# GrokImageCompression/Grok

Measured on AMD Instinct MI355X. Metric: encode Mpixels/s (whole node), 8K RGB HTJ2K lossless, higher is better.
Workload: dtype int16x2 packed (exact: range-proven on the host, int32 fallback); 1 GPU; 8192x8192x3 8-bit RGB, 1 tile, RCT+5/3 lossless HTJ2K, 5 levels, 64x64 blocks (BASELINE metric shape); tiles_per_gpu=1, code_blocks_per_gpu=49152, packed_dwt_levels=4, generator=G2 (SURVEY.md §8d), parallelism=1 GPU, consecutive encodes pipelined (grk_amd_set_pipelining), prewarm_steps=40, input_frames_in_rotation=3

## Files before the change

grok_amd/csrc/context.h:

```cpp
#pragma once
#include "../../include/grok_amd.h"
#include "geometry.h"
#include "kernels.h"
#include "pixel_layout.h"
#include <hip/hip_runtime.h>
#include <cstdio>
#include <cstdlib>
#include <cstring>
#include <string>
#include <vector>
#include <algorithm>
#include <cmath>
#include <atomic>
#include <thread>

using namespace grk_amd;

#pragma GCC visibility push(hidden)
struct DevBuf {
    void* p = nullptr;
    size_t cap = 0;
    hipError_t ensure(size_t n)
    {
        if (n <= cap) return hipSuccess;
// ... 61 lines not shown
    grk_amd_tile_params gp{};
    bool have_geom = false;
    TileGeom geom;
    std::vector<HtBlockDesc> h_desc, h_desc_dec;
    std::vector<uint16_t> dec_qcd;
    std::vector<float> dec_steps;
    std::vector<uint32_t> dec_seg_first;
    std::vector<grk_amd_segment> dec_segs;
    grk_amd_pixel_layout enc_layout{};
    grk_amd_pixel_layout dec_layout{};
    bool dec_upsample = false;
    uint32_t dec_reduce = 0;
    std::vector<uint32_t> red_seg_first;
    std::vector<grk_amd_segment> red_segs;
    DevBuf dec_seg_dev;
    std::vector<HtClassPlan> ht_classes;
    int seq_index = -1;
    int seq_flavour = 0;
    hipStream_t side2 = nullptr; hipEvent_t ev_side2 = nullptr;
    hipStream_t side = nullptr;
    hipEvent_t ev_level0 = nullptr, ev_side = nullptr;
    bool overlap = false;
    static constexpr int kMaxAltSets = 7;
    struct AltSet { DevBuf p1, arena, lengths, offsets, flag, ovf, llA, llB; hipEvent_t ev_side = nullptr, ev_side2 = nullptr; } alts[kMaxAltSets];
    int alt_head = 0;
    int pipe_depth = 2;
    DevBuf ovf;
    bool lds_cap = true;
    bool pipelining = false;
    hipEvent_t ev_main = nullptr;
    bool side_pending = false;
    bool dec_planes16 = true;
    int dwt_pk = 1;
    bool k3_alternate = true;
    uint32_t num_cus = 0;
    uint32_t k3_parity = 0;
    int dwt_xcd = 1;
    bool fuse_egress = true;
    bool planes16 = true;
    DevBuf ht_sel;
    DevBuf energy;
    struct T2State {
        bool valid = false; grk_amd_tile_params p{}; uint32_t order = 0;
        T2Plan plan; uint32_t max_blocks = 0;
        DevBuf packets, pob;
    } t2;
    DevBuf t2_u, t2_h, t2_rel, t2_pkhdr, t2_pkbody, t2_pkdst, t2_lit, t2_litlen, t2_index;
    struct T2Out { DevBuf out, tile_dst, part_len, total; };
    T2Out t2_outs[kMaxAltSets + 1];
    int t2_cur = 0;
    uint64_t t2_out_used = 0;
    std::vector<uint64_t> h_off;
    std::vector<uint32_t> h_len;
    uint32_t last_ntiles = 0;
    uint64_t last_nblocks = 0;
    bool last_h16 = false;
    const uint8_t* last_drops = nullptr;
    DevBuf drops_keep;
    DevBuf rate_L, rate_E, rate_W, rate_drop, rate_res, rate_map, rate_bdrop;
    struct RateState { bool valid = false; RatePlan plan{}; uint64_t nblocks = 0; uint32_t ntiles = 0; std::vector<uint64_t> unit_rows;
                       uint64_t budget = 0;  } rate;
    HostStage stage;
    void* d2h_pin = nullptr; size_t d2h_cap = 0; std::vector<hipEvent_t> d2h_ev;
    hipEvent_t ev_dec_front = nullptr, ev_dec_top = nullptr;
    bool dec_top_pending = false;
    int frame_streams = 1; int fs_parity = 0;
// ... 121 lines not shown
```

grok_amd/csrc/context.hip:

```cpp
#include "context.h"

namespace {
bool create_alt_events(grk_amd_ctx* c)
{
    for (auto& as : c->alts)
        if (hipEventCreateWithFlags(&as.ev_side, hipEventDisableTiming) != hipSuccess ||
            hipEventCreateWithFlags(&as.ev_side2, hipEventDisableTiming) != hipSuccess) return false;
    return true;
}

#ifndef GRK_AMD_OVERLAP_DEFAULT
#define GRK_AMD_OVERLAP_DEFAULT 1
#endif

void drain_timers(grk_amd_ctx* c)
{
    for (auto& t : c->timers) {
        for (auto& pr : t.ev) {
            float ms = 0;
            if (hipEventSynchronize(pr.second) == hipSuccess && hipEventElapsedTime(&ms, pr.first, pr.second) == hipSuccess) {
                t.total_ms += ms; t.launches++;
            }
            (void)hipEventDestroy(pr.first); (void)hipEventDestroy(pr.second);
        }
// ... 175 lines not shown
    c->have_geom = true;
    return GRK_AMD_OK;
}

int stage_enter(grk_amd_ctx* c, const grk_amd_tile_params* p, bool args_ok, bool join, const char* refuse)
{
    if (c && join) { const int jr = join_side(c); if (jr) return jr; }
    if (!c || !p || !args_ok) return GRK_AMD_ERR_INVALID;
    if (refuse) return fail(c, GRK_AMD_ERR_INVALID, refuse);
    HIP_TRY(c, hipSetDevice(c->device), "set device");
    return ensure_geom(c, p);
}

int create_context(int device_id, int verbose, bool decode_only, grk_amd_ctx** out)
{
    if (!out) return GRK_AMD_ERR_INVALID;
    *out = nullptr;
    int n = 0;
    if (hipGetDeviceCount(&n) != hipSuccess || n <= 0) return GRK_AMD_ERR_NO_DEVICE;
    if (device_id < 0 || device_id >= n) return GRK_AMD_ERR_INVALID;
    if (hipSetDevice(device_id) != hipSuccess) return GRK_AMD_ERR_NO_DEVICE;
    auto* c = new grk_amd_ctx();
    c->device = device_id; c->verbose = verbose;
    { int cus = 0; if (hipDeviceGetAttribute(&cus, hipDeviceAttributeMultiprocessorCount, device_id) == hipSuccess && cus > 0) c->num_cus = (uint32_t)cus; }
    if (hipStreamCreateWithFlags(&c->stream, hipStreamNonBlocking) != hipSuccess) { delete c; return GRK_AMD_ERR_NO_DEVICE; }
    c->own_stream = true;
    {
        int least = 0, greatest = 0;
        (void)hipDeviceGetStreamPriorityRange(&least, &greatest);
        if (const char* e16 = getenv("GRK_AMD_PLANES16")) c->planes16 = atoi(e16) != 0;
        if (const char* ef = getenv("GRK_AMD_FUSE_EGRESS")) c->fuse_egress = atoi(ef) != 0;
        if (const char* ex = getenv("GRK_AMD_DWT_XCD")) c->dwt_xcd = atoi(ex) != 0;
        if (const char* ex = getenv("GRK_AMD_DWT_PK")) c->dwt_pk = atoi(ex) != 0;
        if (const char* ek = getenv("GRK_AMD_K3_ALT")) c->k3_alternate = atoi(ek) != 0;
        if (const char* ed = getenv("GRK_AMD_DEC_PLANES16")) c->dec_planes16 = atoi(ed) != 0;
        if (const char* el = getenv("GRK_AMD_LDS_CAP")) c->lds_cap = atoi(el) != 0;
        if (const char* ef2 = getenv("GRK_AMD_FRAME_STREAMS")) c->frame_streams = atoi(ef2);
        if (const char* et = getenv("GRK_AMD_T1_LANES")) c->t1_lanes = atoi(et);
        if (const char* ey = getenv("GRK_AMD_T1_SYNC")) c->t1_pass_sync = atoi(ey) != 0;
        if (const char* ep = getenv("GRK_AMD_STREAM_PROBE")) c->stream_probe = atoi(ep);
        c->side_priority = least;
        const char* e = getenv("GRK_AMD_OVERLAP");
        c->overlap = e ? atoi(e) != 0 : GRK_AMD_OVERLAP_DEFAULT;
        if (hipStreamCreateWithPriority(&c->side, hipStreamNonBlocking, least) != hipSuccess ||
            (!decode_only && hipStreamCreateWithPriority(&c->side2, hipStreamNonBlocking, least) != hipSuccess) ||
            hipEventCreateWithFlags(&c->ev_side2, hipEventDisableTiming) != hipSuccess ||
            !create_alt_events(c) ||
            hipEventCreateWithFlags(&c->ev_level0, hipEventDisableTiming) != hipSuccess ||
            hipEventCreateWithFlags(&c->ev_side, hipEventDisableTiming) != hipSuccess) {
            c->side = nullptr; c->overlap = false;
        }
    }
    *out = c;
    return GRK_AMD_OK;
}

extern "C" {
const char* grk_amd_version(void) { return "grok_amd 0.1 (gfx950)"; }

int grk_amd_create(int device_id, int verbose, grk_amd_ctx** out) { return create_context(device_id, verbose, false, out); }

void grk_amd_destroy(grk_amd_ctx* c)
{
    if (!c) return;
    for (grk_amd_ctx* k : c->dec_kids) grk_amd_destroy(k);
    c->dec_kids.clear();
// ... 180 lines not shown
```

grok_amd/csrc/dwt_instances.h:

```cpp
#pragma once
#include <cstdint>

namespace grk_amd {

struct LevelPart { uint32_t comp0, zdiv, nc; };
inline bool     level_has_triple(bool mct, uint32_t ncomp) { return mct && ncomp >= 3; }
inline uint32_t level_part_count(bool mct, uint32_t ncomp) { return level_has_triple(mct, ncomp) ? ncomp - 2 : 1; }
inline LevelPart level_part(bool mct, uint32_t ncomp, uint32_t i)
{
    if (!level_has_triple(mct, ncomp)) return LevelPart{0, ncomp, 1};
    return i == 0 ? LevelPart{0, 1, 3} : LevelPart{i + 2, 1, 1};
}
inline uint32_t level_part_zslots(bool mct, uint32_t ncomp) { return level_has_triple(mct, ncomp) ? 1u : ncomp; }

inline uint32_t row_segment_pairs(uint64_t strips, uint32_t row_pairs, uint32_t zslots, uint32_t min_wgs)
{
    uint32_t seg = 64;
    while (seg > 8 && strips * ((row_pairs + seg - 1) / seg) * zslots < min_wgs) seg >>= 1;
    return seg;
}

struct DwtKey {
    bool f97; uint8_t nc, px; bool h16, gen, str;
    constexpr uint32_t code() const { return (uint32_t)f97 | nc << 1 | px << 4 | (uint32_t)h16 << 6 | (uint32_t)gen << 7 | (uint32_t)str << 8; }
};
struct DwtPkKey {
    uint8_t nc, px; uint16_t nt; uint8_t ch;
    constexpr uint32_t code() const { return nc | px << 3 | ch << 5 | (uint32_t)nt << 8; }
};
struct IdwtKey {
    bool f97; uint8_t nc, pxo; bool h16, str;
    constexpr uint32_t code() const { return (uint32_t)f97 | nc << 1 | pxo << 4 | (uint32_t)h16 << 6 | (uint32_t)str << 7; }
};
struct IdwtPkKey {
    uint8_t nc, pxo, ch;
    constexpr uint32_t code() const { return nc | pxo << 3 | ch << 5; }
};
struct EgressKey {
    uint8_t bytes, nc; bool str;
    constexpr uint32_t code() const { return bytes | nc << 3 | (uint32_t)str << 6; }
};
struct DwtInstance  { bool packed; DwtKey k; DwtPkKey pk; };
struct IdwtInstance { bool packed; IdwtKey k; IdwtPkKey pk; uint32_t grid_x; };

#define GRK_DWT_INSTANCES(X)                                                                      \
    X(true, 1, 0, false, true, false) X(false, 1, 0, true, true, false) X(false, 1, 0, false, true, false)                       \
    X(true, 3, 1, false, true, true) X(true, 3, 2, false, true, true) X(true, 1, 1, false, true, true) X(true, 1, 2, false, true, true) \
    X(false, 3, 1, true, true, true) X(false, 1, 1, true, true, true)                                                             \
    X(false, 3, 1, false, true, true) X(false, 3, 2, false, true, true) X(false, 1, 1, false, true, true) X(false, 1, 2, false, true, true) \
    X(true, 3, 1, false, false, false) X(true, 3, 1, false, true, false) X(true, 3, 2, false, false, false) X(true, 3, 2, false, true, false) \
    X(true, 1, 1, false, false, false) X(true, 1, 1, false, true, false) X(true, 1, 2, false, false, false) X(true, 1, 2, false, true, false) \
    X(false, 3, 1, true, true, false) X(false, 1, 1, true, true, false)                                                           \
    X(false, 3, 1, false, false, false) X(false, 3, 1, false, true, false) X(false, 3, 2, false, false, false) X(false, 3, 2, false, true, false) \
    X(false, 1, 1, false, false, false) X(false, 1, 1, false, true, false) X(false, 1, 2, false, false, false) X(false, 1, 2, false, true, false)
#define GRK_DWT_PK_INSTANCES(X)                                                                               \
    X(1, 0, 128, 0) X(1, 0, 256, 0)                                                                                               \
    X(1, 1, 128, 1) X(1, 1, 256, 1) X(3, 1, 128, 3) X(3, 1, 256, 3) X(1, 1, 128, 3) X(1, 1, 256, 3)                               \
    X(3, 1, 128, 4) X(3, 1, 256, 4) X(1, 1, 128, 4) X(1, 1, 256, 4)                                                               \
    X(3, 1, 128, 0) X(1, 1, 128, 0) X(3, 1, 256, 0) X(1, 1, 256, 0)
#define GRK_IDWT_INSTANCES(X)                                                                         \
    X(true, 1, 0, false, false) X(false, 1, 0, true, false) X(false, 1, 0, false, false)                                          \
    X(true, 3, 1, false, true) X(true, 3, 2, false, true) X(true, 1, 1, false, true) X(true, 1, 2, false, true)                   \
    X(true, 3, 1, false, false) X(true, 3, 2, false, false) X(true, 1, 1, false, false) X(true, 1, 2, false, false)               \
    X(false, 3, 1, true, true) X(false, 3, 2, true, true) X(false, 1, 1, true, true) X(false, 1, 2, true, true)                   \
    X(false, 3, 1, false, true) X(false, 3, 2, false, true) X(false, 1, 1, false, true) X(false, 1, 2, false, true)               \
    X(false, 3, 1, true, false) X(false, 3, 2, true, false) X(false, 1, 1, true, false) X(false, 1, 2, true, false)               \
    X(false, 3, 1, false, false) X(false, 3, 2, false, false) X(false, 1, 1, false, false) X(false, 1, 2, false, false)
#define GRK_IDWT_PK_INSTANCES(X)                                                                                 \
    X(1, 0, 0) X(1, 1, 1) X(3, 1, 3) X(3, 1, 4) X(3, 1, 0) X(1, 1, 0)
#define GRK_EGRESS_INSTANCES(X)                                                                               \
    X(1, 1, true) X(1, 2, true) X(1, 3, true) X(1, 4, true) X(2, 1, true) X(2, 2, true) X(2, 3, true) X(2, 4, true)               \
    X(1, 1, false) X(1, 2, false) X(1, 3, false) X(1, 4, false) X(2, 1, false) X(2, 2, false) X(2, 3, false) X(2, 4, false)       \
    X(4, 1, false) X(4, 2, false) X(4, 3, false) X(4, 4, false)

#define GRK_INSTANCE_ROW(...) {__VA_ARGS__},
inline constexpr DwtKey    kDwtInstances[]    = {GRK_DWT_INSTANCES(GRK_INSTANCE_ROW)};
inline constexpr DwtPkKey  kDwtPkInstances[]  = {GRK_DWT_PK_INSTANCES(GRK_INSTANCE_ROW)};
inline constexpr IdwtKey   kIdwtInstances[]   = {GRK_IDWT_INSTANCES(GRK_INSTANCE_ROW)};
inline constexpr IdwtPkKey kIdwtPkInstances[] = {GRK_IDWT_PK_INSTANCES(GRK_INSTANCE_ROW)};
inline constexpr EgressKey kEgressInstances[] = {GRK_EGRESS_INSTANCES(GRK_INSTANCE_ROW)};

}
```

grok_amd/csrc/encode.hip:

```cpp
#include "context.h"

namespace {
int encode_layout(grk_amd_ctx* c, uint32_t ntiles, PixelLayout& px)
{
    const char* why = "";
    if (!resolve_pixel_layout(c->geom.p, &c->enc_layout, 0, 0, ntiles, px, &why)) return fail(c, GRK_AMD_ERR_INVALID, why);
    return GRK_AMD_OK;
}

int run_ingest(grk_amd_ctx* c, uint32_t ntiles, const void* d_pixels, void* d_planes, const PixelLayout& px)
{
    const TileGeom& g = c->geom;
    const SampleRange r = sample_range(g.p);
    IngestArgs a{};
    set_px_in(a, px);
    a.pixels = d_pixels; a.planes = (int32_t*)d_planes;
    a.w = g.p.tile_w; a.h = g.p.tile_h; a.stride = g.stride; a.pitch = g.plane_elems;
    a.ncomp = g.p.num_comps; a.ntiles = ntiles;
    a.bytes_per_sample = r.bytes;
    a.dc = r.dc; a.sext = r.sext;
    a.mct = g.p.mct; a.irreversible = g.p.irreversible;
    ScopedTimer t(c, 0);
    HIP_TRY(c, launch_ingest(a, c->stream), "launch ingest");
    return GRK_AMD_OK;
// ... 49 lines not shown
int run_dwt(grk_amd_ctx* c, uint32_t nplanes, void* d_in, void* d_out, const void* d_pixels = nullptr, uint32_t ntiles = 0,
            const HtArgs* overlap_ht = nullptr, bool h16 = false, const PixelLayout* px = nullptr)
{
    const TileGeom& g = c->geom;
    const uint32_t L = g.p.num_levels;
    if (L == 0) {
        HIP_TRY(c, hipMemcpyAsync(d_out, d_in, (size_t)nplanes * g.plane_elems * 4, hipMemcpyDeviceToDevice, c->stream), "copy planes");
        return GRK_AMD_OK;
    }
    { const int rc = ensure_ll(c, nplanes); if (rc) return rc; }
    ScopedTimer t(c, 1);
    const SampleRange r = sample_range(g.p);
    for (uint32_t l = 0; l < L; ++l) {
        DwtLevelArgs a{};
        a.cw = level_geom(g, l).w; a.ch = level_geom(g, l).h;
        a.px = level_geom(g, l).x0 & 1u; a.py = level_geom(g, l).y0 & 1u;
        const LLPlane from = ll_plane(c, l, d_in, d_out), to = ll_plane(c, l + 1, d_in, d_out);
        a.in = (const int32_t*)from.p; a.in_stride = from.stride; a.in_pitch = from.pitch;
        a.mallat = (int32_t*)d_out; a.m_stride = g.stride; a.m_pitch = g.plane_elems;
        a.ll = (int32_t*)to.p; a.ll_stride = to.stride; a.ll_pitch = to.pitch;
        a.nplanes = nplanes;
        a.irreversible = g.p.irreversible;
        a.h16 = h16 ? 1 : 0;
        a.pk = h16 && c->dwt_pk && pk16_level_ok(g.p, l);
        a.xcd = c->dwt_xcd;
        if (l == 0 && d_pixels && px && px->lay) {
            set_px_in(a, *px); a.px_chan = px->channels;
        }
        const bool fused = l == 0 && d_pixels;
        const uint32_t zslots = fused ? ntiles * level_part_zslots(g.p.mct != 0, g.p.num_comps) : nplanes;
        const DwtLevelShape shape = plan_dwt_level(DwtLevelDesc{a.cw, a.ch, a.px, a.py, a.in_stride, a.m_stride, a.h16 != 0, a.pk != 0,
                                                                a.irreversible != 0, a.px_lay, a.px_chan, a.px_row, zslots, fused, r.bytes});
        a.seg_pairs = shape.seg_pairs;
        if (a.cw == 0 || a.ch == 0) {
        } else if (fused) {
            a.pixels = d_pixels; a.px_bytes = r.bytes;
            a.alloc_reset = c->pend_alloc; a.alloc_chunk_units = c->pend_alloc_units; c->pend_alloc = nullptr;
            a.dc = r.dc; a.sext = r.sext;
            HIP_TRY(c, launch_dwt_level0_fused(a, shape, ntiles, g.p.num_comps, g.p.mct, c->stream), "launch fused dwt level 0");
            if (c->want_px_event) HIP_TRY(c, hipEventRecord(c->ev_px, c->stream), "record the pixels' last read");
        } else {
            HIP_TRY(c, launch_dwt_level(a, shape, c->stream), "launch dwt level");
        }
        if (overlap_ht && (l == 0 || l + 1 == L)) {
            HIP_TRY(c, hipEventRecord(c->ev_level0, c->stream), "record level");
            const int rc = launch_ht_at(c, *overlap_ht, true, l == 0 ? HtPoint::AfterLevel0 : HtPoint::AfterLastLevel, L == 1);
            if (rc) return rc;
            if (l + 1 == L) {
                HIP_TRY(c, hipEventRecord(c->ev_side, c->side), "record side stream");
                HIP_TRY(c, hipEventRecord(c->ev_side2, c->side2), "record side stream 2");
            }
        }
    }
    return GRK_AMD_OK;
}

int run_ht(grk_amd_ctx* c, HtArgs a, bool overlapped = false, bool room = false)
{
    a.room = room ? 1 : 0;
    {
        ScopedTimer t(c, 2);
        if (!overlapped) HIP_TRY(c, launch_ht_alloc_init(a, c->stream), "reset arena allocator");
        const int rc = launch_ht_at(c, a, overlapped, HtPoint::RunHt, false);
        if (rc) return rc;
    }
    if (overlapped) {
        c->side_pending = true;
        if (!c->pipelining) { const int jr = join_side(c); if (jr) return jr; }
    }
    c->last_ntiles = a.ntiles;
    c->last_nblocks = (uint64_t)a.blocks_per_tile * a.ntiles;
    c->last_drops = nullptr;
    return GRK_AMD_OK;
}
}

int ht_encode_drops(grk_amd_ctx* c, uint32_t ntiles, const void* d_mallat, bool h16, const uint8_t* d_drops)
{
    HtArgs a;
    const int rc = make_ht_args(c, ntiles, d_mallat, h16, a); if (rc) return rc;
    const HtDropPlan dp = plan_ht_drop_instance(a.irreversible != 0, a.h16 != 0);
    if (!dp.ok) return fail(c, GRK_AMD_ERR_INVALID, "no encode keeps irreversible int16 planes");
    const uint64_t nblocks = (uint64_t)a.blocks_per_tile * a.ntiles;
    HIP_TRY(c, c->drops_keep.ensure(nblocks), "alloc drops copy");
    HIP_TRY(c, hipMemcpyAsync(c->drops_keep.p, d_drops, nblocks, hipMemcpyDeviceToDevice, c->stream), "keep the drops");
// ... 333 lines not shown
```

grok_amd/csrc/encode_constants.h:

```cpp
#pragma once
#include <cstddef>
#include <cstdint>

#if defined(__HIP_DEVICE_COMPILE__) || defined(__HIPCC__)
#define GRK_ENC_FN __host__ __device__ inline
#else
#define GRK_ENC_FN inline
#endif

namespace grk_amd {

constexpr uint32_t kHtMaxClasses = 24;
#ifndef GRK_HT_ALLOC_REGIONS
#define GRK_HT_ALLOC_REGIONS 64
#endif
constexpr uint32_t kHtAllocRegions = GRK_HT_ALLOC_REGIONS;
constexpr uint32_t kHtAllocChunk = 64u << 10;
constexpr uint32_t kHtAllocChunkSmall = 32u << 10;
constexpr size_t   kHtAllocBytes = 256u * (1u + kHtAllocRegions);
constexpr uint32_t kHtBlocksPerRegion = 64;
constexpr uint32_t kHtSmallJobBlocks = 16384;
constexpr size_t   kLdsPerCu = 160u << 10;
constexpr size_t   kMaxWavesPerCu = 32;
constexpr size_t   kLdsFor16Waves = 10240;

constexpr uint32_t kHtDropSkip = 0xFFu;
constexpr uint32_t kRateDefaultDrop = 6;
constexpr uint32_t kRateMaxDrop = 12;
constexpr uint32_t kRateMaxCand = kRateMaxDrop + 2;
constexpr uint32_t kRateAllocThreads = 1024;
constexpr uint32_t kRateBisectSteps = 40;
constexpr uint64_t kRateMaxBlocks = 0x7FFFFFFFull;
constexpr uint32_t kRateMaxRounds = 4;

constexpr uint64_t kFrameStreamSamples = 16ull << 20;

constexpr uint32_t kDwtStripCols = 448;
constexpr int      kPkLaneCols = 4;
constexpr uint32_t kPkNarrowCols = 2048;
GRK_ENC_FN uint32_t pk_strip_cols(uint32_t cw, uint32_t nt)
{
    const uint32_t most = ((nt - 2u) * kPkLaneCols) & ~63u;
    const uint32_t n = (cw + most - 1) / most;
    const uint32_t even = ((cw + n - 1) / n + 63u) & ~63u;
    return even < most ? even : most;
}
constexpr uint32_t kDwtMinWgsPacked = 2048;
constexpr uint32_t kDwtMinWgs = 4096;

}
```

grok_amd/csrc/encode_plan.cpp:

```cpp
#include "encode_plan.h"
#include <algorithm>

namespace grk_amd {

HtClasses plan_ht_classes(const TileGeom& g, uint32_t ncomp, bool lds_cap)
{
    HtClasses out;
    const uint32_t bpc = (uint32_t)g.blocks_comp0.size();
    auto add_class = [&](HtRole role, int top, int big) {
        HtClassPlan cl{0, 0, 0, 0, 0, (uint32_t)out.sel.size(), role};
        uint32_t hist[64] = {0};
        for (uint32_t i = 0; i < ncomp * bpc; ++i) {
            const grk_amd_block& b = g.blocks_comp0[i % bpc];
            if (top >= 0 && (int)(b.res == g.p.num_levels && g.p.num_levels >= 1) != top) continue;
            const uint32_t w = b.x1 - b.x0, h = b.y1 - b.y0;
            const uint32_t samples = w * h, quads = ((w + 1u) / 2u) * ((h + 1u) / 2u);
            if (big >= 0 && (int)(ht_lds_bytes(samples, quads, b.kmax) > kLdsFor16Waves) != big) continue;
            cl.count++;
            cl.max_kmax = std::max<uint32_t>(cl.max_kmax, b.kmax);
            cl.max_samples = std::max(cl.max_samples, samples);
            cl.max_quads = std::max(cl.max_quads, quads);
            hist[b.kmax & 63u] += samples;
            out.sel.push_back(i);
        }
// ... 154 lines not shown
    } else if (d.px_lay != 0) {
        in.packed = !d.irreversible && px == 1 && s.packed;
        const uint8_t ch = d.px_chan == 1 ? 1 : d.px_chan == 3 ? 3 : 4;
        in.pk = DwtPkKey{ch == 1 ? (uint8_t)1 : nc, 1, (uint16_t)s.lanes, ch};
        in.k = DwtKey{d.irreversible, nc, px, h16 && px == 1, true, true};
    } else {
        in.packed = !d.irreversible && px == 1 && s.packed;
        in.pk = DwtPkKey{nc, 1, (uint16_t)s.lanes, 0};
        if (h16 && px == 1) in.k = DwtKey{false, nc, 1, true, true, false};
        else                in.k = DwtKey{d.irreversible, nc, px, false, !s.all_fast, false};
    }
    return in;
}

DwtLevelShape plan_dwt_level(const DwtLevelDesc& d)
{
    DwtLevelShape s{};
    const bool near = (uint64_t)d.m_stride * d.ch < (1ull << 31) && (uint64_t)d.cw * d.ch < (1ull << 31) && (uint64_t)d.in_stride * d.ch < (1ull << 31);
    const bool lay = d.px_lay == 0 || (d.px_lay == 2 && (d.px_chan == 1 || d.px_chan == 3 || d.px_chan == 4) && d.px_row * d.ch < (1ull << 31));
    s.packed = d.h16 && d.pk && !d.irreversible && (d.px | d.py) == 0 && (d.cw & 3u) == 0 && d.cw >= 256u &&
               d.ch >= 16 && (d.ch & 1u) == 0 && near && lay;
    s.lanes = s.packed && d.cw <= kPkNarrowCols ? 128u : 256u;
    s.strip_cols = s.packed ? pk_strip_cols(d.cw, s.lanes) : kDwtStripCols;
    s.all_fast = (d.px | d.py) == 0 && (d.cw & 1u) == 0 && d.cw >= 4 && d.ch >= 16 && (d.ch & 1u) == 0;
    const uint32_t row_pairs = (d.ch + d.py + 1) >> 1;
    s.grid_x = (uint32_t)(((uint64_t)d.cw + d.px + s.strip_cols - 1) / s.strip_cols);
    s.seg_pairs = row_segment_pairs(s.grid_x, row_pairs, d.zslots, d.pk ? kDwtMinWgsPacked : kDwtMinWgs);
    s.grid_y = (row_pairs + s.seg_pairs - 1) / s.seg_pairs;
    s.inst[0] = dwt_instance(d, s, 1);
    if (d.fused) s.inst[1] = dwt_instance(d, s, 3);
    return s;
}

}
```

grok_amd/csrc/encode_plan.h:

```cpp
#pragma once
#include "dwt_instances.h"
#include "encode_constants.h"
#include "geometry.h"
#include <cstddef>
#include <cstdint>
#include <vector>

#pragma GCC visibility push(hidden)
namespace grk_amd {

enum class HtRole : uint8_t { Top, Rest, All, TopSmall, TopBig, RestSmall, RestBig };
struct HtClassPlan {
    uint32_t count;
    uint32_t max_kmax, max_samples, max_quads;
    uint32_t cap_kmax;
    uint32_t first;
    HtRole role;
};
struct HtClasses {
    std::vector<uint32_t> sel;
    std::vector<HtClassPlan> classes;
};
HtClasses plan_ht_classes(const TileGeom& g, uint32_t ncomp, bool lds_cap);

// ... 67 lines not shown
    bool overlap, pipelining; int frame_streams; bool planes16;
    bool have_side, have_side2;
    bool on_device;
    uint32_t px_align;
    uint64_t samples;
};
struct Route {
    bool fused;
    bool overlap;
    bool frame_stream;
    bool h16;
};
Route plan_route(const grk_amd_tile_params& p, const RouteIn& in);

struct DwtLevelDesc {
    uint32_t cw, ch, px, py;
    uint32_t in_stride, m_stride;
    bool h16, pk, irreversible;
    uint32_t px_lay, px_chan; uint64_t px_row;
    uint32_t zslots;
    bool fused; uint32_t px_bytes;
};
struct DwtLevelShape {
    bool packed;
    uint32_t lanes;
    uint32_t strip_cols;
    bool all_fast;
    uint32_t seg_pairs;
    uint32_t grid_x, grid_y;
    DwtInstance inst[2];
};
DwtLevelShape plan_dwt_level(const DwtLevelDesc& d);

}
#pragma GCC visibility pop
```

grok_amd/csrc/kernels.h:

```cpp
#pragma once
#include <cstdint>
#include <hip/hip_runtime.h>
#include "geometry.h"
#include "decode_constants.h"
#include "encode_constants.h"
#include "encode_plan.h"
#include "decode_plan.h"

namespace grk_amd {

struct IngestArgs {
    const void* pixels;
    int32_t*    planes;
    uint32_t w, h, stride;
    uint64_t pitch;
    uint32_t ncomp, ntiles;
    uint32_t bytes_per_sample;
    int32_t  dc;
    int32_t  sext;
    int      mct;
    int      irreversible;
    uint32_t px_lay, px_xstep;
    uint64_t px_row, px_kstep, px_tile;
};
hipError_t launch_ingest(const IngestArgs& a, hipStream_t s);

struct DwtLevelArgs {
    const int32_t* in;  uint32_t in_stride;  uint64_t in_pitch;
    int32_t* ll;        uint32_t ll_stride;  uint64_t ll_pitch;
    int32_t* mallat;    uint32_t m_stride;   uint64_t m_pitch;
    uint32_t cw, ch;
    uint32_t px, py;
    uint32_t nplanes;
    uint32_t seg_pairs;
    int      irreversible;
    const void* pixels;
    uint32_t px_bytes;
    int32_t  dc;
    int32_t  sext;
    uint32_t ncomp;
    uint32_t comp0, zdiv;
    unsigned long long* alloc_reset; uint32_t alloc_chunk_units;
    int      h16;
    int      xcd;
    int      pk;
    uint32_t px_lay, px_chan, px_xstep;
    uint64_t px_row, px_kstep, px_tile;
};
hipError_t launch_dwt_level(const DwtLevelArgs& a, const DwtLevelShape& sh, hipStream_t s);
hipError_t launch_dwt_level0_fused(const DwtLevelArgs& a0, const DwtLevelShape& sh, uint32_t ntiles, uint32_t ncomp, int mct, hipStream_t s);

struct HtBlockDesc {
    uint32_t px, py;
    uint16_t w, h;
    uint16_t comp;
    uint8_t  kmax;
    uint8_t  pad;
    float    inv_step;
};
struct HtClass {
    const uint32_t* sel;
    uint32_t count;
    uint32_t max_kmax, max_samples, max_quads;
    uint32_t ovf_base;
    uint32_t cap_kmax;
};
struct HtArgs {
    const int32_t* mallat; uint32_t stride; uint64_t pitch;
    int h16;
    int room;
    const HtBlockDesc* blocks; uint32_t blocks_per_tile; uint32_t ncomp; uint32_t ntiles;
    uint8_t*  arena; uint64_t arena_bytes;
    unsigned long long* alloc;
    uint32_t* lengths;
    unsigned long long* offsets;
    const uint32_t* sel; uint32_t sel_count;
    uint32_t* ovf_list; uint32_t ovf_base;
    HtClass classes[kHtMaxClasses]; uint32_t num_classes;
    uint32_t region_mask;
    uint32_t chunk_units;
    const uint32_t* vlc_tab;
    int irreversible;
};
// ... 213 lines not shown
```

grok_amd/csrc/kernels_dwt.hip:

```cpp
#include "kernels.h"
#include "dwt_common.h"
#include "pk16.h"
#include <type_traits>

namespace grk_amd {

namespace {

constexpr int   kThreads  = 256;
constexpr int   kCols     = 2 * kThreads;
constexpr int   kHalo     = 4;
constexpr int   kOutCols  = (int)kDwtStripCols;
constexpr int   kOutPairs = kOutCols / 2;
static_assert(kOutCols <= kCols - 2 * kHalo && kOutCols % 2 == 0, "strip does not fit the staged line");

struct V53 {
    int32_t xe, dp;
    __device__ __forceinline__ void init(int32_t x_even) { xe = x_even; dp = 0; }
    __device__ __forceinline__ void step(int32_t x1, int32_t x2, int32_t& s, int32_t& d)
    {
        d = x1 - ((xe + x2) >> 1);
        s = xe + ((dp + d + 2) >> 2);
        xe = x2; dp = d;
    }
// ... 484 lines not shown
        for (int k = 0; k < NC; ++k) {
            const uint32_t ju = (uint32_t)j;
            const uint32_t lrow = __builtin_amdgcn_readfirstlane(ju * a.ll_stride * 2u),
                           mlo = __builtin_amdgcn_readfirstlane(ju * a.m_stride * 2u),
                           mhi = __builtin_amdgcn_readfirstlane((sh + ju) * a.m_stride * 2u);
            __builtin_amdgcn_raw_buffer_store_b32(o[k][0], r_ll[k], oc, lrow, 0);
            const __amdgpu_buffer_rsrc_t rm = r_mp[k];
            __builtin_amdgcn_raw_buffer_store_b32(o[k][1], rm, oc, mhi, 0);
            __builtin_amdgcn_raw_buffer_store_b32(o[k][2], rm, oc + 2u * sw, mlo, 0);
            __builtin_amdgcn_raw_buffer_store_b32(o[k][3], rm, oc + 2u * sw, mhi, 0);
        }
    };
    auto no_stores = [&]() {
    #pragma unroll
        for (int k = 0; k < 4 * NC; ++k) __builtin_amdgcn_raw_buffer_store_b32(0u, r_none, oc + 64 * k, 0, 0);
    };
    const int32_t i_end = J1 - 1;
    uint32_t o[NC][4];
    int32_t ii = J0, jp;
    vstep(J0 - 1, ra1, ra2); no_stores();
    __builtin_amdgcn_sched_barrier(0);
    vstep(ii, rb1, rb2); no_stores(); hphase(0, o); jp = ii; ++ii;
    __builtin_amdgcn_sched_barrier(0);
    while (ii + 1 <= i_end) {
        vstep(ii, ra1, ra2); store_out(jp, o); hphase(1, o); jp = ii; ++ii;
        __builtin_amdgcn_sched_barrier(0);
        vstep(ii, rb1, rb2); store_out(jp, o); hphase(0, o); jp = ii; ++ii;
        __builtin_amdgcn_sched_barrier(0);
    }
    if (ii <= i_end) { vstep(ii, ra1, ra2); store_out(jp, o); hphase(1, o); jp = ii; }
    store_out(jp, o);
}

}

static hipError_t launch_dwt_instance(const DwtInstance& in, dim3 grid, const DwtLevelArgs& a, hipStream_t s)
{
    if (in.packed) {
        switch (in.pk.code()) {
#define GRK_X(NC, PX, NT, CH) case DwtPkKey{NC, PX, NT, CH}.code(): hipLaunchKernelGGL((dwt53_pk_kernel<NC, PX, NT, CH>), grid, dim3(NT), 0, s, a); break;
        GRK_DWT_PK_INSTANCES(GRK_X)
#undef GRK_X
        default: return hipErrorInvalidValue;
        }
    } else {
        switch (in.k.code()) {
#define GRK_X(F97, NC, PX, H16, GEN, STR) case DwtKey{F97, NC, PX, H16, GEN, STR}.code(): hipLaunchKernelGGL((dwt_level_kernel<F97, NC, PX, H16, GEN, STR>), grid, dim3(kThreads), 0, s, a); break;
        GRK_DWT_INSTANCES(GRK_X)
#undef GRK_X
        default: return hipErrorInvalidValue;
        }
    }
    return hipSuccess;
}

hipError_t launch_dwt_level(const DwtLevelArgs& a, const DwtLevelShape& sh, hipStream_t s)
{
    const hipError_t e = launch_dwt_instance(sh.inst[0], dim3(sh.grid_x, sh.grid_y, a.nplanes), a, s);
    return e != hipSuccess ? e : hipGetLastError();
}

hipError_t launch_dwt_level0_fused(const DwtLevelArgs& a0, const DwtLevelShape& sh, uint32_t ntiles, uint32_t ncomp, int mct, hipStream_t s)
{
    for (uint32_t i = 0; i < level_part_count(mct != 0, ncomp); ++i) {
        const LevelPart part = level_part(mct != 0, ncomp, i);
        DwtLevelArgs a = a0;
        a.comp0 = part.comp0; a.zdiv = part.zdiv; a.ncomp = ncomp;
        if (part.comp0 != 0) a.alloc_reset = nullptr;
        const hipError_t e = launch_dwt_instance(sh.inst[part.nc == 3], dim3(sh.grid_x, sh.grid_y, ntiles * part.zdiv), a, s);
        if (e != hipSuccess) return e;
    }
    return hipGetLastError();
}

}
```

grok_amd/csrc/pk16.h:

```cpp
#pragma once
#include <hip/hip_runtime.h>
#include <cstdint>

namespace grk_amd {

typedef short pk16 __attribute__((ext_vector_type(2)));
__device__ __forceinline__ pk16 as_pk(uint32_t v) { return __builtin_bit_cast(pk16, v); }
__device__ __forceinline__ uint32_t as_u32(pk16 v) { return __builtin_bit_cast(uint32_t, v); }
typedef unsigned int u32x2 __attribute__((ext_vector_type(2)));
typedef unsigned int u32x3 __attribute__((ext_vector_type(3)));
typedef unsigned int u32x4 __attribute__((ext_vector_type(4)));

constexpr uint32_t kSelLoLo = 0x05040100u;
constexpr uint32_t kSelHiHi = 0x07060302u;

__device__ __forceinline__ __amdgpu_buffer_rsrc_t buffer_from(const void* p, bool none = false)
{
    return __builtin_amdgcn_make_buffer_rsrc(const_cast<void*>(p), 0, none ? 0 : -1, 0x00020000);
}

constexpr int32_t kPkDecodeBound = 2047;

}
```

Measured before the change: 201,800 Mpixels/s.

## Fuse DWT levels 0 and 1 into one packed int16 kernel for RGB 8-bit

Adds a fused kernel that does RCT plus the first 5/3 DWT level from 8-bit pixels and immediately runs the second level's vertical and horizontal lifting on the LL output held in LDS. Level 1's detail bands go to the mallat buffer and its LL goes to the level-2 plane. The level-0 LL is never written to or re-read from global memory, and one kernel launch is saved. The price is extra LDS, larger row segments capped at 32, dummy stores to keep the schedule uniform, and a more complex halo and boundary path. The path is on by default and selected only for reversible, h16, 3-component, unshifted shapes.

```diff
diff --git a/grok_amd/csrc/context.h b/grok_amd/csrc/context.h
--- a/grok_amd/csrc/context.h
+++ b/grok_amd/csrc/context.h
@@ -117,6 +117,7 @@
     bool side_pending = false;
     bool dec_planes16 = true;
     int dwt_pk = 1;
+    int dwt_pair = 1;
     bool k3_alternate = true;
     uint32_t num_cus = 0;
     uint32_t k3_parity = 0;
diff --git a/grok_amd/csrc/context.hip b/grok_amd/csrc/context.hip
--- a/grok_amd/csrc/context.hip
+++ b/grok_amd/csrc/context.hip
@@ -231,6 +231,7 @@
         if (const char* ef = getenv("GRK_AMD_FUSE_EGRESS")) c->fuse_egress = atoi(ef) != 0;
         if (const char* ex = getenv("GRK_AMD_DWT_XCD")) c->dwt_xcd = atoi(ex) != 0;
         if (const char* ex = getenv("GRK_AMD_DWT_PK")) c->dwt_pk = atoi(ex) != 0;
+        if (const char* ex = getenv("GRK_AMD_DWT_PAIR")) c->dwt_pair = atoi(ex) != 0;
         if (const char* ek = getenv("GRK_AMD_K3_ALT")) c->k3_alternate = atoi(ek) != 0;
         if (const char* ed = getenv("GRK_AMD_DEC_PLANES16")) c->dec_planes16 = atoi(ed) != 0;
         if (const char* el = getenv("GRK_AMD_LDS_CAP")) c->lds_cap = atoi(el) != 0;
diff --git a/grok_amd/csrc/dwt_instances.h b/grok_amd/csrc/dwt_instances.h
--- a/grok_amd/csrc/dwt_instances.h
+++ b/grok_amd/csrc/dwt_instances.h
@@ -27,6 +27,10 @@
 struct DwtPkKey {
     uint8_t nc, px; uint16_t nt; uint8_t ch;
     constexpr uint32_t code() const { return nc | px << 3 | ch << 5 | (uint32_t)nt << 8; }
+};
+struct DwtPairKey {
+    uint8_t nc, px; uint16_t nt;
+    constexpr uint32_t code() const { return nc | px << 3 | (uint32_t)nt << 8; }
 };
 struct IdwtKey {
     bool f97; uint8_t nc, pxo; bool h16, str;
@@ -58,6 +62,8 @@
     X(1, 1, 128, 1) X(1, 1, 256, 1) X(3, 1, 128, 3) X(3, 1, 256, 3) X(1, 1, 128, 3) X(1, 1, 256, 3)                               \
     X(3, 1, 128, 4) X(3, 1, 256, 4) X(1, 1, 128, 4) X(1, 1, 256, 4)                                                               \
     X(3, 1, 128, 0) X(1, 1, 128, 0) X(3, 1, 256, 0) X(1, 1, 256, 0)
+#define GRK_DWT_PAIR_INSTANCES(X)                                                                                 \
+    X(3, 1, 128) X(3, 1, 256)
 #define GRK_IDWT_INSTANCES(X)                                                                         \
     X(true, 1, 0, false, false) X(false, 1, 0, true, false) X(false, 1, 0, false, false)                                          \
     X(true, 3, 1, false, true) X(true, 3, 2, false, true) X(true, 1, 1, false, true) X(true, 1, 2, false, true)                   \
@@ -76,6 +82,7 @@
 #define GRK_INSTANCE_ROW(...) {__VA_ARGS__},
 inline constexpr DwtKey    kDwtInstances[]    = {GRK_DWT_INSTANCES(GRK_INSTANCE_ROW)};
 inline constexpr DwtPkKey  kDwtPkInstances[]  = {GRK_DWT_PK_INSTANCES(GRK_INSTANCE_ROW)};
+inline constexpr DwtPairKey kDwtPairInstances[] = {GRK_DWT_PAIR_INSTANCES(GRK_INSTANCE_ROW)};
 inline constexpr IdwtKey   kIdwtInstances[]   = {GRK_IDWT_INSTANCES(GRK_INSTANCE_ROW)};
 inline constexpr IdwtPkKey kIdwtPkInstances[] = {GRK_IDWT_PK_INSTANCES(GRK_INSTANCE_ROW)};
 inline constexpr EgressKey kEgressInstances[] = {GRK_EGRESS_INSTANCES(GRK_INSTANCE_ROW)};
diff --git a/grok_amd/csrc/encode.hip b/grok_amd/csrc/encode.hip
--- a/grok_amd/csrc/encode.hip
+++ b/grok_amd/csrc/encode.hip
@@ -105,7 +105,19 @@
         const DwtLevelShape shape = plan_dwt_level(DwtLevelDesc{a.cw, a.ch, a.px, a.py, a.in_stride, a.m_stride, a.h16 != 0, a.pk != 0,
                                                                 a.irreversible != 0, a.px_lay, a.px_chan, a.px_row, zslots, fused, r.bytes});
         a.seg_pairs = shape.seg_pairs;
+        uint32_t last = l;
+        const DwtPairShape pair = plan_dwt_pair_at(g, l, DwtPairAsk{c->dwt_pair != 0, c->dwt_pk != 0, fused, h16, a.px_lay, a.px_chan, a.px_row,
+                                                                    r.bytes, to.stride, ntiles});
         if (a.cw == 0 || a.ch == 0) {
+        } else if (pair.ok) {
+            const LLPlane to2 = ll_plane(c, l + 2, d_in, d_out);
+            a.ll2 = (int32_t*)to2.p; a.ll2_stride = to2.stride; a.ll2_pitch = to2.pitch;
+            a.pixels = d_pixels; a.px_bytes = r.bytes;
+            a.alloc_reset = c->pend_alloc; a.alloc_chunk_units = c->pend_alloc_units; c->pend_alloc = nullptr;
+            a.dc = r.dc; a.sext = r.sext;
+            HIP_TRY(c, launch_dwt_pair(a, pair, ntiles, c->stream), "launch fused dwt levels 0 and 1");
+            if (c->want_px_event) HIP_TRY(c, hipEventRecord(c->ev_px, c->stream), "record the pixels' last read");
+            last = l + 1;
         } else if (fused) {
             a.pixels = d_pixels; a.px_bytes = r.bytes;
             a.alloc_reset = c->pend_alloc; a.alloc_chunk_units = c->pend_alloc_units; c->pend_alloc = nullptr;
@@ -115,15 +127,16 @@
         } else {
             HIP_TRY(c, launch_dwt_level(a, shape, c->stream), "launch dwt level");
         }
-        if (overlap_ht && (l == 0 || l + 1 == L)) {
+        if (overlap_ht && (l == 0 || last + 1 == L)) {
             HIP_TRY(c, hipEventRecord(c->ev_level0, c->stream), "record level");
-            const int rc = launch_ht_at(c, *overlap_ht, true, l == 0 ? HtPoint::AfterLevel0 : HtPoint::AfterLastLevel, L == 1);
+            const int rc = launch_ht_at(c, *overlap_ht, true, l == 0 ? HtPoint::AfterLevel0 : HtPoint::AfterLastLevel, l == 0 && last + 1 == L);
             if (rc) return rc;
-            if (l + 1 == L) {
+            if (last + 1 == L) {
                 HIP_TRY(c, hipEventRecord(c->ev_side, c->side), "record side stream");
                 HIP_TRY(c, hipEventRecord(c->ev_side2, c->side2), "record side stream 2");
             }
         }
+        l = last;
     }
     return GRK_AMD_OK;
 }
diff --git a/grok_amd/csrc/encode_constants.h b/grok_amd/csrc/encode_constants.h
--- a/grok_amd/csrc/encode_constants.h
+++ b/grok_amd/csrc/encode_constants.h
@@ -47,5 +47,14 @@
 }
 constexpr uint32_t kDwtMinWgsPacked = 2048;
 constexpr uint32_t kDwtMinWgs = 4096;
+struct DwtPairRows { int32_t store0, store1, first, last, low0, low1; };
+GRK_ENC_FN DwtPairRows dwt_pair_rows(uint32_t seg, uint32_t seg_pairs, uint32_t ch)
+{
+    const int32_t sh = (int32_t)(ch >> 1), j0 = (int32_t)(seg * seg_pairs);
+    const int32_t j1 = j0 + (int32_t)seg_pairs < sh ? j0 + (int32_t)seg_pairs : sh;
+    return DwtPairRows{j0, j1, j0 - 2, j1, j0 >> 1, j1 >> 1};
+}
+constexpr uint32_t kDwtPairMinWgs = 1024;
+constexpr uint32_t kDwtPairMaxSeg = 32;
 
 }
diff --git a/grok_amd/csrc/encode_plan.cpp b/grok_amd/csrc/encode_plan.cpp
--- a/grok_amd/csrc/encode_plan.cpp
+++ b/grok_amd/csrc/encode_plan.cpp
@@ -210,4 +210,39 @@
     return s;
 }
 
-}
+DwtPairShape plan_dwt_pair(const DwtPairDesc& d)
+{
+    DwtPairShape s{};
+    const DwtLevelDesc& u = d.upper;
+    const DwtLevelShape up = plan_dwt_level(u), low = plan_dwt_level(d.lower);
+    const bool levels = up.packed && low.packed && up.inst[1].packed && low.inst[0].packed;
+    const bool pixels = u.fused && u.px_lay == 0 && u.px_bytes == 1 && d.mct && d.ncomp == 3 && u.h16 && !u.irreversible;
+    const bool shape = (u.cw & 7u) == 0 && u.cw >= 512 && (u.ch & 3u) == 0 && u.ch >= 32 && (u.px | u.py | d.lower.px | d.lower.py) == 0 &&
+                       d.lower.cw == u.cw >> 1 && d.lower.ch == u.ch >> 1;
+    const bool near = (uint64_t)u.m_stride * u.ch * 2u < (1ull << 31);
+    if (!(levels && pixels && shape && near && d.ntiles > 0)) return s;
+    s.ok = true;
+    s.lanes = up.lanes;
+    s.strip_cols = up.strip_cols;
+    s.grid_x = up.grid_x;
+    s.seg_pairs = std::min(kDwtPairMaxSeg, row_segment_pairs(s.grid_x, u.ch >> 1, d.ntiles, kDwtPairMinWgs));
+    s.grid_y = ((u.ch >> 1) + s.seg_pairs - 1) / s.seg_pairs;
+    s.inst = DwtPairKey{3, 1, (uint16_t)s.lanes};
+    return s;
+}
+
+DwtPairShape plan_dwt_pair_at(const TileGeom& g, uint32_t l, const DwtPairAsk& q)
+{
+    if (!q.pair || !q.fused || l != 0 || l + 1 >= g.p.num_levels) return DwtPairShape{};
+    const ResGeom& g0 = level_geom(g, l);
+    const ResGeom& g1 = level_geom(g, l + 1);
+    const bool irrev = g.p.irreversible != 0;
+    const uint32_t zslots = q.ntiles * level_part_zslots(g.p.mct != 0, g.p.num_comps);
+    const DwtLevelDesc upper{g0.w, g0.h, g0.x0 & 1u, g0.y0 & 1u, g.stride, g.stride, q.h16, q.h16 && q.dwt_pk && pk16_level_ok(g.p, l), irrev,
+                             q.px_lay, q.px_chan, q.px_row, zslots, true, q.px_bytes};
+    const DwtLevelDesc lower{g1.w, g1.h, g1.x0 & 1u, g1.y0 & 1u, q.mid_stride, g.stride, q.h16, q.h16 && q.dwt_pk && pk16_level_ok(g.p, l + 1), irrev,
+                             0, 0, 0, q.ntiles * g.p.num_comps, false, q.px_bytes};
+    return plan_dwt_pair(DwtPairDesc{upper, lower, g.p.mct != 0, g.p.num_comps, q.ntiles});
+}
+
+}
diff --git a/grok_amd/csrc/encode_plan.h b/grok_amd/csrc/encode_plan.h
--- a/grok_amd/csrc/encode_plan.h
+++ b/grok_amd/csrc/encode_plan.h
@@ -123,5 +123,17 @@
 };
 DwtLevelShape plan_dwt_level(const DwtLevelDesc& d);
 
+struct DwtPairDesc { DwtLevelDesc upper, lower; bool mct; uint32_t ncomp, ntiles; };
+struct DwtPairShape {
+    bool ok;
+    uint32_t lanes, strip_cols;
+    uint32_t seg_pairs;
+    uint32_t grid_x, grid_y;
+    DwtPairKey inst;
+};
+DwtPairShape plan_dwt_pair(const DwtPairDesc& d);
+struct DwtPairAsk { bool pair, dwt_pk, fused, h16; uint32_t px_lay, px_chan; uint64_t px_row; uint32_t px_bytes, mid_stride, ntiles; };
+DwtPairShape plan_dwt_pair_at(const TileGeom& g, uint32_t l, const DwtPairAsk& q);
+
 }
 #pragma GCC visibility pop
diff --git a/grok_amd/csrc/kernels.h b/grok_amd/csrc/kernels.h
--- a/grok_amd/csrc/kernels.h
+++ b/grok_amd/csrc/kernels.h
@@ -46,9 +46,11 @@
     int      pk;
     uint32_t px_lay, px_chan, px_xstep;
     uint64_t px_row, px_kstep, px_tile;
+    int32_t* ll2;       uint32_t ll2_stride; uint64_t ll2_pitch;
 };
 hipError_t launch_dwt_level(const DwtLevelArgs& a, const DwtLevelShape& sh, hipStream_t s);
 hipError_t launch_dwt_level0_fused(const DwtLevelArgs& a0, const DwtLevelShape& sh, uint32_t ntiles, uint32_t ncomp, int mct, hipStream_t s);
+hipError_t launch_dwt_pair(const DwtLevelArgs& a0, const DwtPairShape& sh, uint32_t ntiles, hipStream_t s);
 
 struct HtBlockDesc {
     uint32_t px, py;
diff --git a/grok_amd/csrc/kernels_dwt.hip b/grok_amd/csrc/kernels_dwt.hip
--- a/grok_amd/csrc/kernels_dwt.hip
+++ b/grok_amd/csrc/kernels_dwt.hip
@@ -540,6 +540,213 @@
     store_out(jp, o);
 }
 
+namespace pair {
+
+constexpr uint32_t kDropOff = 0x80000000u;
+
+template <int NC, int PX, int NT>
+__global__ __launch_bounds__(NT) void dwt53_pk_kernel(DwtLevelArgs a)
+{
+    static_assert(PX == 1, "8-bit pixels in component planes");
+    static_assert((((NT - 4) * kPkLaneCols) & ~63) == (((NT - 2) * kPkLaneCols) & ~63), "pk_strip_cols leaves room for two halo lanes a side");
+    __builtin_amdgcn_s_setprio(3);
+    constexpr int kPkCols = NT * kPkLaneCols;
+    __shared__ __attribute__((aligned(16))) uint32_t line[2][NC][kPkCols];
+    __shared__ __attribute__((aligned(16))) uint32_t line1[NC][2 * NT];
+
+    const uint32_t t = threadIdx.x;
+    uint32_t bx = blockIdx.x, by = blockIdx.y, bz = blockIdx.z;
+    if (a.alloc_reset && (bx | by | bz) == 0) ht_alloc_reset(a.alloc_reset, a.alloc_chunk_units, threadIdx.x, blockDim.x);
+    if (a.xcd) {
+        const uint32_t gx = gridDim.x, gy = gridDim.y, total = gx * gy * gridDim.z;
+        const uint32_t id = bx + gx * (by + gy * bz);
+        const uint32_t q = total >> 3, r = total & 7u, k = id & 7u;
+        const uint32_t lid = k * q + min(k, r) + (id >> 3);
+        bx = lid % gx; by = (lid / gx) % gy; bz = lid / (gx * gy);
+    }
+    const uint32_t cw = a.cw, ch = a.ch;
+    const uint32_t sw = cw >> 1, sh = ch >> 1, sw1 = cw >> 2, sh1 = ch >> 2;
+    const uint32_t scols = pk_strip_cols(cw, NT), slanes = scols / kPkLaneCols;
+
+    const uint32_t plane0 = (bz / a.zdiv) * a.ncomp + a.comp0 + (bz % a.zdiv);
+    int16_t* l2 = reinterpret_cast<int16_t*>(a.ll2) + (size_t)plane0 * a.ll2_pitch;
+    int16_t* mp = reinterpret_cast<int16_t*>(a.mallat) + (size_t)plane0 * a.m_pitch;
+    const size_t comp_px = (size_t)cw * ch;
+    const uint8_t* pix = reinterpret_cast<const uint8_t*>(a.pixels) + (size_t)plane0 * comp_px;
+
+    const uint32_t grp = t < slanes ? t + 2u : (t < slanes + 2u ? t - slanes : (t < slanes + 4u ? t : 2u));
+    const int32_t c0 = (int32_t)(bx * scols) - 2 * kPkHalo + (int32_t)(grp * kPkLaneCols);
+    const bool rev = c0 < 0 || c0 >= (int32_t)cw;
+    int32_t lo = c0 < 0 ? -c0 - 3 : (c0 >= (int32_t)cw ? 2 * ((int32_t)cw - 1) - c0 - 3 : c0);
+    lo = max(0, min(lo, (int32_t)cw - kPkLaneCols));
+    const uint32_t lane_off = (uint32_t)lo;
+    const uint32_t selA = rev ? 0x0c020c03u : 0x0c010c00u, selB = rev ? 0x0c000c01u : 0x0c030c02u;
+    const pk16 dc2 = as_pk((uint32_t)a.dc * 0x10001u);
+
+    __amdgpu_buffer_rsrc_t r_in[NC], r_l2[NC], r_mp[NC];
+    const uint32_t m_bytes = (uint32_t)min((unsigned long long)a.m_pitch * 2u, 0x7fffffffull);
+    const uint32_t l2_bytes = (uint32_t)min((unsigned long long)a.ll2_pitch * 2u, 0x7fffffffull);
+    #pragma unroll
+    for (int k = 0; k < NC; ++k) {
+        r_in[k] = buffer_from(pix + (size_t)k * comp_px);
+        r_l2[k] = buffer_of(l2 + (size_t)k * a.ll2_pitch, l2_bytes);
+        r_mp[k] = buffer_of(mp + (size_t)k * a.m_pitch, m_bytes);
+    }
+    __amdgpu_buffer_rsrc_t r_none = buffer_from(a.mallat, true);
+
+    const DwtPairRows rows = dwt_pair_rows(by, a.seg_pairs, ch);
+    const int32_t J0 = rows.store0;
+    const int32_t Q0 = rows.first;
+    const int32_t n1 = rows.low1 - rows.low0;
+
+    struct Raw { uint32_t v[NC]; };
+    auto fetch_row = [&](int32_t r, Raw& q) {
+        const uint32_t rr = mirror_row<true>(r, ch);
+    #pragma unroll
+        for (int k = 0; k < NC; ++k) q.v[k] = __builtin_amdgcn_raw_buffer_load_b32(r_in[k], lane_off, rr * cw, kPkLoadAux);
+    };
+    auto convert = [&](const Raw& q, pk16 (&va)[NC], pk16 (&vb)[NC]) {
+        pk16 xa[NC], xb[NC];
+    #pragma unroll
+        for (int k = 0; k < NC; ++k) {
+            xa[k] = as_pk(__builtin_amdgcn_perm(0u, q.v[k], selA));
+            xb[k] = as_pk(__builtin_amdgcn_perm(0u, q.v[k], selB));
+        }
+        if constexpr (NC == 3) {
+            const pk16 cba = xa[2] - xa[1], cra = xa[0] - xa[1], cbb = xb[2] - xb[1], crb = xb[0] - xb[1];
+            va[0] = xa[1] + ((cba + cra) >> 2) - dc2; va[1] = cba; va[2] = cra;
+            vb[0] = xb[1] + ((cbb + crb) >> 2) - dc2; vb[1] = cbb; vb[2] = crb;
+        } else { va[0] = xa[0] - dc2; vb[0] = xb[0] - dc2; }
+    };
+
+    V53pk colA[NC], colB[NC], col1[NC];
+    {
+        Raw q; pk16 xa[NC], xb[NC];
+        fetch_row(2 * (Q0 - 1), q);
+        convert(q, xa, xb);
+    #pragma unroll
+        for (int k = 0; k < NC; ++k) { colA[k].init(xa[k]); colB[k].init(xb[k]); }
+    }
+    Raw ra1, ra2, rb1, rb2;
+    fetch_row(2 * Q0 - 1, ra1); fetch_row(2 * Q0, ra2);
+    fetch_row(2 * Q0 + 1, rb1); fetch_row(2 * Q0 + 2, rb2);
+
+    const uint32_t nv = min(slanes, (sw - bx * (scols / 2) + 1u) >> 1);
+    const bool last_strip = (bx + 1u) * scols >= cw;
+    const uint32_t hg = t < slanes ? min(t, nv - 1u) + 2u : (t == slanes ? 1u : (t == slanes + 1u ? nv + 2u : 2u));
+    const uint32_t hc = hg * kPkLaneCols;
+    const uint32_t oc = t < slanes ? (bx * (scols / 2) + (hg - 2u) * 2u) * 2u : kDropOff;
+    const uint32_t w1 = 2u * hg + ((last_strip && t == slanes + 1u) ? 2u : 0u);
+    const uint32_t x1slot = (last_strip && t < slanes && hg == nv + 1u) ? 2u * hg + 2u : w1;
+    const uint32_t nv1 = nv >> 1;
+    const uint32_t hc1 = 4u * min(t, nv1 - 1u) + 4u;
+    const uint32_t oc1 = t < nv1 ? (bx * (scols / 4) + t * 2u) * 2u : kDropOff;
+
+    pk16 sA[NC], dA[NC], sB[NC], dB[NC];
+    auto vstep = [&](int32_t ii, Raw& r1, Raw& r2) {
+        pk16 x1a[NC], x1b[NC], x2a[NC], x2b[NC];
+        convert(r1, x1a, x1b); convert(r2, x2a, x2b);
+        fetch_row(2 * ii + 5, r1); fetch_row(2 * ii + 6, r2);
+    #pragma unroll
+        for (int k = 0; k < NC; ++k) { colA[k].step(x1a[k], x2a[k], sA[k], dA[k]); colB[k].step(x1b[k], x2b[k], sB[k], dB[k]); }
+    };
+    auto stencil = [&](const uint32_t* w, uint32_t (&o)[4]) {
+        const uint2 m = *reinterpret_cast<const uint2*>(w - 2);
+        const uint4 c = *reinterpret_cast<const uint4*>(w);
+        const pk16 m2 = as_pk(m.x), m1 = as_pk(m.y), c0 = as_pk(c.x), c1 = as_pk(c.y), c2 = as_pk(c.z), c3 = as_pk(c.w),
+                   p4 = as_pk(w[4]);
+        const pk16 dm = m1 - ((m2 + c0) >> 1);
+        const pk16 d0 = c1 - ((c0 + c2) >> 1);
+        const pk16 d1 = c3 - ((c2 + p4) >> 1);
+        const pk16 s0 = c0 + ((dm + d0 + (pk16)(2)) >> 2);
+        const pk16 s1 = c2 + ((d0 + d1 + (pk16)(2)) >> 2);
+        o[0] = __builtin_amdgcn_perm(as_u32(s1), as_u32(s0), kSelLoLo);
+        o[1] = __builtin_amdgcn_perm(as_u32(s1), as_u32(s0), kSelHiHi);
+        o[2] = __builtin_amdgcn_perm(as_u32(d1), as_u32(d0), kSelLoLo);
+        o[3] = __builtin_amdgcn_perm(as_u32(d1), as_u32(d0), kSelHiHi);
+    };
+    auto lower_out = [&](int32_t j1, bool valid) {
+        const uint32_t ju = (uint32_t)j1;
+        const uint32_t lrow = __builtin_amdgcn_readfirstlane(ju * a.ll2_stride * 2u),
+                       mlo = __builtin_amdgcn_readfirstlane(ju * a.m_stride * 2u),
+                       mhi = __builtin_amdgcn_readfirstlane((sh1 + ju) * a.m_stride * 2u);
+    #pragma unroll
+        for (int k = 0; k < NC; ++k) {
+            uint32_t o1[4];
+            stencil(&line1[k][hc1], o1);
+            const __amdgpu_buffer_rsrc_t rl = valid ? r_l2[k] : r_none, rm = valid ? r_mp[k] : r_none;
+            __builtin_amdgcn_raw_buffer_store_b32(o1[0], rl, oc1, lrow, 0);
+            __builtin_amdgcn_raw_buffer_store_b32(o1[1], rm, oc1, mhi, 0);
+            __builtin_amdgcn_raw_buffer_store_b32(o1[2], rm, oc1 + 2u * sw1, mlo, 0);
+            __builtin_amdgcn_raw_buffer_store_b32(o1[3], rm, oc1 + 2u * sw1, mhi, 0);
+        }
+    };
+    auto hphase = [&](int par, uint32_t (&o)[NC][4]) {
+    #pragma unroll
+        for (int k = 0; k < NC; ++k) {
+            uint4 w;
+            w.x = __builtin_amdgcn_perm(as_u32(dA[k]), as_u32(sA[k]), kSelLoLo);
+            w.y = __builtin_amdgcn_perm(as_u32(dA[k]), as_u32(sA[k]), kSelHiHi);
+            w.z = __builtin_amdgcn_perm(as_u32(dB[k]), as_u32(sB[k]), kSelLoLo);
+            w.w = __builtin_amdgcn_perm(as_u32(dB[k]), as_u32(sB[k]), kSelHiHi);
+            *reinterpret_cast<uint4*>(&line[par][k][grp * kPkLaneCols]) = w;
+        }
+        __syncthreads();
+    #pragma unroll
+        for (int k = 0; k < NC; ++k) stencil(&line[par][k][hc], o[k]);
+    };
+    auto store_out = [&](int32_t j, const uint32_t (&o)[NC][4], bool valid) {
+        const uint32_t ju = (uint32_t)j;
+        const uint32_t mlo = __builtin_amdgcn_readfirstlane(ju * a.m_stride * 2u),
+                       mhi = __builtin_amdgcn_readfirstlane((sh + ju) * a.m_stride * 2u);
+    #pragma unroll
+        for (int k = 0; k < NC; ++k) {
+            const __amdgpu_buffer_rsrc_t rm = valid ? r_mp[k] : r_none;
+            __builtin_amdgcn_raw_buffer_store_b32(o[k][1], rm, oc, mhi, 0);
+            __builtin_amdgcn_raw_buffer_store_b32(o[k][2], rm, oc + 2u * sw, mlo, 0);
+            __builtin_amdgcn_raw_buffer_store_b32(o[k][3], rm, oc + 2u * sw, mhi, 0);
+        }
+    };
+    pk16 x1[NC];
+    auto lower_vstep = [&](const uint32_t (&o)[NC][4], bool last) {
+    #pragma unroll
+        for (int k = 0; k < NC; ++k) {
+            const pk16 x2 = last ? col1[k].xe : as_pk(o[k][0]);
+            pk16 s, d;
+            col1[k].step(x1[k], x2, s, d);
+            uint2 w;
+            w.x = __builtin_amdgcn_perm(as_u32(d), as_u32(s), kSelLoLo);
+            w.y = __builtin_amdgcn_perm(as_u32(d), as_u32(s), kSelHiHi);
+            *reinterpret_cast<uint2*>(&line1[k][w1]) = w;
+            line1[k][x1slot] = w.x;
+        }
+    };
+    auto no_stores = [&](int n) {
+    #pragma unroll
+        for (int k = 0; k < n; ++k) __builtin_amdgcn_raw_buffer_store_b32(0u, r_none, 64 * k, 0, 0);
+    };
+    uint32_t o[NC][4];
+    vstep(Q0 - 1, ra1, ra2); no_stores(7 * NC);
+    __builtin_amdgcn_sched_barrier(0);
+    vstep(Q0, rb1, rb2); no_stores(3 * NC); hphase(0, o);
+    #pragma unroll
+    for (int k = 0; k < NC; ++k) col1[k].init(as_pk(o[k][0]));
+    __builtin_amdgcn_sched_barrier(0);
+    for (int32_t it = 0; it <= n1; ++it) {
+        const int32_t A = Q0 + 1 + 2 * it, B = A + 1;
+        vstep(A, ra1, ra2); store_out(B - 2, o, it >= 1); hphase(1, o); lower_out((J0 >> 1) + it - 2, it >= 2);
+    #pragma unroll
+        for (int k = 0; k < NC; ++k) x1[k] = as_pk(o[k][0]);
+        __builtin_amdgcn_sched_barrier(0);
+        vstep(B, rb1, rb2); store_out(A, o, it >= 1); hphase(0, o); lower_vstep(o, B == (int32_t)sh);
+        __builtin_amdgcn_sched_barrier(0);
+    }
+    __syncthreads();
+    lower_out((J0 >> 1) + n1 - 1, true);
+}
+
+}
+
 }
 
 static hipError_t launch_dwt_instance(const DwtInstance& in, dim3 grid, const DwtLevelArgs& a, hipStream_t s)
@@ -581,4 +788,19 @@
     return hipGetLastError();
 }
 
-}
+hipError_t launch_dwt_pair(const DwtLevelArgs& a0, const DwtPairShape& sh, uint32_t ntiles, hipStream_t s)
+{
+    if (!sh.ok) return hipErrorInvalidValue;
+    DwtLevelArgs a = a0;
+    a.comp0 = 0; a.zdiv = 1; a.ncomp = 3; a.seg_pairs = sh.seg_pairs;
+    const dim3 grid(sh.grid_x, sh.grid_y, ntiles);
+    switch (sh.inst.code()) {
+#define GRK_X(NC, PX, NT) case DwtPairKey{NC, PX, NT}.code(): hipLaunchKernelGGL((pair::dwt53_pk_kernel<NC, PX, NT>), grid, dim3(NT), 0, s, a); break;
+    GRK_DWT_PAIR_INSTANCES(GRK_X)
+#undef GRK_X
+    default: return hipErrorInvalidValue;
+    }
+    return hipGetLastError();
+}
+
+}
diff --git a/grok_amd/csrc/pk16.h b/grok_amd/csrc/pk16.h
--- a/grok_amd/csrc/pk16.h
+++ b/grok_amd/csrc/pk16.h
@@ -18,6 +18,10 @@
 {
     return __builtin_amdgcn_make_buffer_rsrc(const_cast<void*>(p), 0, none ? 0 : -1, 0x00020000);
 }
+__device__ __forceinline__ __amdgpu_buffer_rsrc_t buffer_of(const void* p, uint32_t bytes)
+{
+    return __builtin_amdgcn_make_buffer_rsrc(const_cast<void*>(p), 0, (int)bytes, 0x00020000);
+}
 
 constexpr int32_t kPkDecodeBound = 2047;
 
```

Measured after the change: 216,800 Mpixels/s (median of 6 runs). 7.4% higher.
